# google-deepmind/pycolab

Hardware: NVIDIA H100
Metric: env_steps_per_sec (higher is better)
Workload: dtype u8

## Files before the change

pycolab_b200/csrc/pcl_kernels.cuh:

```cuda
#pragma once

#include <cuda_runtime.h>
#include <stdint.h>
#include <string.h>

#include "../../include/pcl.h"

namespace pcl {

struct CropParams {
  int B, H, W, pitch, S;
  pcl_crop_spec crop;
  const int32_t* sprites;
  int32_t* plot;
  int32_t* state;
  const uint8_t* board;
  uint8_t* out;
  const uint8_t* curtains[PCL_MAX_TRACK];
  uint32_t cols_recip;
};

struct StepParams {
  int B, H, W, pitch;
  int PH, PW, PWW;
  int BW;
  int S, D;
  int auto_reset;
  int mode;
  int actions_per_env;
  int margin[PCL_MAX_DRAPES][2];
  uint8_t sprite_char[PCL_MAX_SPRITES];
  uint8_t drape_char[PCL_MAX_DRAPES];
  uint32_t impassable[PCL_MAX_SPRITES][4];
  int confined[PCL_MAX_SPRITES];
  int egocentric[PCL_MAX_SPRITES];
  int drape_kind[PCL_MAX_DRAPES];
  int program_arg[8];
  int n_scroll_groups;
  int sprite_group[PCL_MAX_SPRITES];
  int drape_group[PCL_MAX_DRAPES];
  int n_groups;
  int group_len[PCL_MAX_SPRITES + PCL_MAX_DRAPES];
  uint8_t group_chars[PCL_MAX_SPRITES + PCL_MAX_DRAPES];
  pcl_state st;
  pcl_outputs out;
  const int32_t* actions;
  const uint8_t* env_mask;
  int has_cropper;
  CropParams cropper;
  const int32_t* code;
  uint8_t* backdrop_live;
  const uint32_t* derived[2];
  int64_t derived_bstride[2];
  int32_t* render_key;
  uint32_t board_epoch;
};

template <typename... Params, typename... Args>
cudaError_t launch_pdl(void (*kern)(Params...), int grid, int block, size_t smem, cudaStream_t s,
                       Args... args) {
  cudaLaunchConfig_t cfg = {};
  cfg.gridDim = dim3(grid); cfg.blockDim = dim3(block); cfg.dynamicSmemBytes = smem; cfg.stream = s;
  cudaLaunchAttribute attr[1];
  attr[0].id = cudaLaunchAttributeProgrammaticStreamSerialization;
  attr[0].val.programmaticStreamSerializationAllowed = 1;
  cfg.attrs = attr; cfg.numAttrs = 1;
  return cudaLaunchKernelEx(&cfg, kern, args...);
}

inline cudaError_t launch_step(void (*kern)(StepParams), const StepParams& p, int warps,
                               size_t smem, cudaStream_t s, bool pdl = false) {
  if (smem > 48 * 1024) {
    cudaError_t e = cudaFuncSetAttribute(kern, cudaFuncAttributeMaxDynamicSharedMemorySize, (int)smem);
    if (e != cudaSuccess) return e;
  }
  const int grid = (p.B + warps - 1) / warps;
  if (pdl) return launch_pdl(kern, grid, warps * 32, smem, s, p);
  kern<<<grid, warps * 32, smem, s>>>(p);
  return cudaGetLastError();
}

enum class CurtainAt { kNone, kBits, kPatternWindow, kStaleWindow };

struct Program {
  int (*check_spec)(const pcl_spec&);
  int (*check_state)(const pcl_spec&, const pcl_state&);
  CurtainAt (*curtain)(const pcl_spec&, int drape);
  cudaError_t (*launch)(const StepParams&, cudaStream_t);
  int (*actions_per_env)(const pcl_spec&);
  bool float_reward;
  bool crop_epilogue;
  bool scroll_groups;
  int (*check_code)(const pcl_spec&, const int32_t* words, int n_words);
  bool float_reward_arg0;
  int (*derive)(const pcl_spec&, const pcl_state&, int batch, StepParams* base, void** owned);
};
extern const Program kScrollyMaze, kWarehouse, kMarauders, kFixture, kBetterScrolly, kClassics,
    kAperture, kOrdeal, kHello, kApprehend, kShockwave, kTMaze, kCompiled, kBoxWorld,
    kCuedCatch, kSequenceRecall;

inline bool chars_are(const uint8_t* got, int n, const char* want) {
  if ((int)strlen(want) != n) return false;
  for (int i = 0; i < n; ++i) if (got[i] != (uint8_t)want[i]) return false;
  return true;
}

inline bool set_is(const uint32_t (&got)[4], const char* want) {
  uint32_t m[4] = {0, 0, 0, 0};
  for (const char* c = want; *c; ++c) m[(*c >> 5) & 3] |= 1u << (*c & 31);
  return m[0] == got[0] && m[1] == got[1] && m[2] == got[2] && m[3] == got[3];
}

inline int groups_are(const pcl_spec& s, const char* flat, const int* lens, int n) {
  if (s.n_groups != n) return 0;
  int k = 0;
  for (int g = 0; g < n; ++g) {
    if (s.group_len[g] != lens[g]) return 0;
    for (int i = 0; i < lens[g]; ++i, ++k)
      if (s.group_chars[k] != (uint8_t)flat[k]) return 0;
  }
  return 1;
}

inline bool bit_rows_fit(const pcl_spec& s) { return s.bits_words >= (s.cols + 31) / 32 + 1; }

inline bool margins_fit(const pcl_spec& s, int d) {
  const int mr = s.margins[d][0], mc = s.margins[d][1];
  return !(mr >= 0 && (mc - 1 >= s.cols - mc || mr - 1 >= s.rows - mr));
}

inline CurtainAt curtain_bits(const pcl_spec&, int) { return CurtainAt::kBits; }

struct RenderParams {
  int B, H, W, pitch, S, D;
  const uint8_t* backdrop; int64_t backdrop_bstride;
  const uint8_t* curtains;
  const int32_t* sprites;
  const uint8_t* z_order;
  uint8_t sprite_char[PCL_MAX_SPRITES];
  uint8_t drape_char[PCL_MAX_DRAPES];
  uint8_t* board;
};
cudaError_t launch_render(const RenderParams& p, cudaStream_t s);

#define PCL_MAX_LAYER_CHARS 32
struct LayersParams {
  int B, H, W, pitch, S, D, n_chars;
  uint8_t chars[PCL_MAX_LAYER_CHARS];
  int8_t sprite_of[PCL_MAX_LAYER_CHARS];
  int8_t drape_of[PCL_MAX_LAYER_CHARS];
  const uint32_t* bits[PCL_MAX_DRAPES]; int64_t bits_bstride[PCL_MAX_DRAPES];
  int row_words[PCL_MAX_DRAPES];
  int scrolly[PCL_MAX_DRAPES];
  int per_level[PCL_MAX_DRAPES];
  int stale_slot[PCL_MAX_DRAPES];
  const uint8_t* backdrop; int64_t backdrop_bstride;
  const int32_t* level;
  const int32_t* sprites;
  const int32_t* drapes;
  uint8_t* out;
  int backdrop_per_env;
};
cudaError_t launch_layers(const LayersParams& p, cudaStream_t s);

struct ObserveParams {
  int B, H, W, pitch, depth, dtype;
  int words;
  int64_t stride_b, stride_d, stride_r, stride_c;
  const void* table;
  const uint8_t* valid;
  const uint8_t* board;
  void* out;
  int32_t* unknown;
};
cudaError_t launch_observe(const ObserveParams& p, cudaStream_t s);

cudaError_t launch_crop(const CropParams& p, cudaStream_t s);

struct HandoffParams {
  int n_peers, rank, record_bytes;
  int64_t rows;
  int64_t first_row;
  uint8_t* peer_base[PCL_MAX_PEERS];
  uint32_t* peer_flags[PCL_MAX_PEERS];
  uint8_t* multicast;
  uint32_t* local;
  int n_bufs, lag;
  int signal_kernel;
  pcl_outputs out;
};
cudaError_t launch_crop_handoff(const CropParams& p, const HandoffParams& x, cudaStream_t s);

struct PackParams {
  int B, view_bytes, record_bytes;
  const uint8_t* view;
  pcl_outputs out;
  uint8_t* packed;
  int n_peers;
  int64_t first_row;
  uint8_t* peers[PCL_MAX_PEERS];
};
cudaError_t launch_pack_handoff(const PackParams& p, cudaStream_t s);

}
```

pycolab_b200/csrc/scrolly_maze.cu:

```cuda
#include <algorithm>
#include <new>

#include "pcl_device.cuh"
#include "pcl_kernels.cuh"
#include "pcl_crop.cuh"

namespace pcl {

namespace {

constexpr int kS = 4;
constexpr int kWarpsPerBlock = 4;
constexpr int kRecWords = 64;

__device__ __forceinline__ int action_to_motion(int a) {
  constexpr unsigned kTable = (PCL_M_N) | (PCL_M_S << 4) | (PCL_M_W << 8) | (PCL_M_E << 12) |
                              (PCL_M_STAY << 16);
  return (unsigned)a < 5u ? (int)((kTable >> (4 * a)) & 15u) : PCL_M_NONE;
}

__device__ __forceinline__ void cp_async8(void* smem, const void* gmem) {
  asm volatile("cp.async.ca.shared.global [%0], [%1], 8;\n" ::
               "r"((uint32_t)__cvta_generic_to_shared(smem)), "l"(gmem));
}
__device__ __forceinline__ void cp_async16_l1(void* smem, const void* gmem) {
  asm volatile("cp.async.ca.shared.global [%0], [%1], 16;\n" ::
               "r"((uint32_t)__cvta_generic_to_shared(smem)), "l"(gmem));
}


__device__ __forceinline__ int coin_group_shift(int PH) {
  return 32 - __clz((PH - 1) >> 5);
}

__device__ __forceinline__ uint32_t prmt(uint32_t a, uint32_t b, uint32_t sel) {
  uint32_t d;
  asm("prmt.b32 %0, %1, %2, %3;" : "=r"(d) : "r"(a), "r"(b), "r"(sel));
  return d;
}

__host__ __device__ constexpr int window_words(int W) {
  return W < 2 ? 4 : 2 * ((63 + W + 63) / 64);
}

__host__ __device__ constexpr bool narrow_board(int pitch) { return pitch <= 64; }

constexpr int kKeyStride = 16;
enum { kKeyRecWords = 8, kKeyEpoch = 8, kKeySprites = 9, kKeyWords = kKeySprites + kS };
constexpr uint64_t kKeyRec =
    (uint64_t)(48 + PCL_P_FRAME) | (uint64_t)(32 + PCL_D_CORNER_R) << 8 |
    (uint64_t)(32 + PCL_D_CORNER_C) << 16 | (uint64_t)(40 + PCL_D_CORNER_R) << 24 |
    (uint64_t)(40 + PCL_D_CORNER_C) << 32 | (uint64_t)(40 + PCL_D_AUX0) << 40 |
    (uint64_t)(40 + PCL_D_AUX1) << 48 | (uint64_t)(40 + PCL_D_AUX2) << 56;
static_assert(kKeyWords <= kKeyStride, "the render key outgrew its slot");

enum {
  kNbWall = 0,
  kNbCoin = 32,
  kNbBackdrop = 44,
  kNbStart = 56,
  kNbStale = kNbStart + 4 * kS,
  kNbWords = (kNbStale + 2 + 3) & ~3
};

__host__ __device__ constexpr size_t staging_bytes(int H, int W, int pitch) {
  return (size_t)H * pitch + 2 * ((((size_t)H * window_words(W) * 4) + 15) & ~(size_t)15) +
         (narrow_board(pitch) ? 0 : (((size_t)H * (pitch >> 2) + 15) & ~(size_t)15));
}

__host__ __device__ constexpr size_t warp_smem_bytes(int H, int W, int pitch) {
  return kRecWords * 4 + (staging_bytes(H, W, pitch) > (size_t)kNbWords * 4
                             ? staging_bytes(H, W, pitch) : (size_t)kNbWords * 4);
}

__device__ __forceinline__ void pdl_launch_dependents() {
  asm volatile("griddepcontrol.launch_dependents;" ::: "memory");
}
__device__ __forceinline__ void pdl_wait_prior_grids() {
  asm volatile("griddepcontrol.wait;" ::: "memory");
}

struct SelTable { uint16_t v[256]; };
constexpr SelTable make_sel_table() {
  SelTable t = {};
  for (int idx = 0; idx < 256; ++idx) {
    unsigned sel = 0;
    for (int k = 0; k < 4; ++k) {
      const unsigned nib = ((idx >> (4 + k)) & 1) ? 5u : ((idx >> k) & 1) ? 4u : (unsigned)k;
      sel |= nib << (4 * k);
    }
    t.v[idx] = (uint16_t)sel;
  }
  return t;
}
__device__ __align__(16) const SelTable g_sel = make_sel_table();

#ifdef PCL_STEP_STAMPS
constexpr int kStampEnvs = 8192;
enum {
  kStEntry, kStPrior, kStRecords, kStPatch, kStGroup2, kStWait, kStPatched, kStPaint, kStEnd,
  kStTimeIn, kStTimeOut, kStPath, kStampWords
};
enum { kPathDelta, kPathDeltaPickup, kPathFellBack, kPathFull, kPathRestart };
__device__ uint32_t g_stamps[kStampEnvs][kStampWords];
__device__ __forceinline__ uint32_t global_ns() {
  uint32_t t;
  asm volatile("mov.u32 %0, %%globaltimer_lo;" : "=r"(t));
  return t;
}
__device__ __forceinline__ void stamp(int k, uint32_t v) {
  uint32_t tid, cta;
  asm volatile("mov.u32 %0, %%tid.x;" : "=r"(tid));
  asm volatile("mov.u32 %0, %%ctaid.x;" : "=r"(cta));
  const uint32_t e = cta * kWarpsPerBlock + (tid >> 5);
  if ((tid & 31) == 0 && e < (uint32_t)kStampEnvs) g_stamps[e][k] = v;
}
#define PCL_STAMP(k) stamp(k, (uint32_t)clock())
#define PCL_STAMP_TIME(k) stamp(k, global_ns())
#define PCL_STAMP_PATH(v) stamp(kStPath, (uint32_t)(v))
#else
#define PCL_STAMP(k) do {} while (0)
#define PCL_STAMP_TIME(k) do {} while (0)
#define PCL_STAMP_PATH(v) do {} while (0)
#endif

constexpr size_t kMaxBlockSmem = 227 * 1024 - 2048;

static_assert(8 * (kWarpsPerBlock * (warp_smem_bytes(64, 64, 64) + sizeof(SelTable)) + 1024) <=
                  228 * 1024,
              "a 64x64 scrolly_maze block no longer fits 8 times per SM");
static_assert(warp_smem_bytes(1, 1, 16) == kRecWords * 4 + kNbWords * 4,
              "delta rendering's scratch must fit a warp's region on the smallest board");
static_assert(kMaxBlockSmem + kWarpsPerBlock * sizeof(SelTable) == 227 * 1024,
              "kMaxBlockSmem must leave room for the static selector tables");

__device__ __forceinline__ unsigned blocked3x3(int vrow, int vcol, int r0, int c0, unsigned field,
                                               int H, int W, bool p_vis, int p_row, int p_col) {
  const int br = vrow - r0 + 1, bc = vcol - c0 + 1;
  if ((unsigned)br > 2u || (unsigned)bc > 2u) return 0u;
  unsigned colmask = 0;
#pragma unroll
  for (int i = 0; i < 3; ++i) colmask |= ((unsigned)(vcol - 1 + i) < (unsigned)W ? 1u : 0u) << i;
  unsigned blk = 0;
#pragma unroll
  for (int j = 0; j < 3; ++j) {
    unsigned bits = (field >> ((br + j) * 5 + bc)) & colmask;
    if ((unsigned)(vrow - 1 + j) >= (unsigned)H) bits = 0;
    blk |= bits << (3 * j);
  }
  const int dr = p_row - vrow + 1, dc = p_col - vcol + 1;
  if (p_vis && (unsigned)dr <= 2u && (unsigned)dc <= 2u) blk &= ~(1u << (dr * 3 + dc));
  return blk;
}

__device__ __forceinline__ int legal_motions(unsigned b) {
  const unsigned nw = b & 1u, n = (b >> 1) & 1u, ne = (b >> 2) & 1u, w = (b >> 3) & 1u,
                 e = (b >> 5) & 1u, sw = (b >> 6) & 1u, s = (b >> 7) & 1u, se = (b >> 8) & 1u;
  const unsigned blocked = n | ((ne | (n & e)) << 1) | (e << 2) | ((se | (s & e)) << 3) |
                           (s << 4) | ((sw | (s & w)) << 5) | (w << 6) | ((nw | (n & w)) << 7);
  return (int)((~blocked & 0xffu) | (1u << PCL_M_STAY));
}

__device__ __forceinline__ void scrolly_move_p(Drape& d, const ScrollyCfg& cfg, int motion,
                                               Plot& plot, int p_row, int p_col, int p_permit,
                                               int p_permit_frame) {
  if (d.last_frame < plot.frame) {
    d.last_frame = plot.frame;
    d.pre_r = d.corner_r; d.pre_c = d.corner_c;
  }
  const int dr = motion_dr(motion), dc = motion_dc(motion);
  if (plot.order_frame == plot.frame) {
    if (dr != plot.order_r && dc != plot.order_c) plot.error |= PCL_ENV_ERR_ORDER_MISMATCH;
    d.corner_r += plot.order_r; d.corner_c += plot.order_c;
    return;
  }
  if (motion == PCL_M_STAY) return;
  const bool ego = plot.ego_mask & 1;
  const bool possible = !ego || (p_permit_frame == plot.frame && ((p_permit >> motion) & 1));
  int orr, occ;
  if (!cfg.have_margins) {
    if (!possible) return;
    const int nr = d.corner_r + dr, nc = d.corner_c + dc;
    orr = (0 <= nr && nr <= cfg.limit_r) ? dr : 0;
    occ = (0 <= nc && nc <= cfg.limit_c) ? dc : 0;
  } else {
    if (!ego) return;
    const int nr = p_row + dr, nc = p_col + dc;
    const bool want_v = (p_row > nr && nr <= cfg.m_north) || (p_row < nr && nr >= cfg.m_south);
    const bool want_h = (p_col > nc && nc <= cfg.m_west) || (p_col < nc && nc >= cfg.m_east);
    if (!(want_v || want_h)) return;
    orr = want_v ? dr : 0; occ = want_h ? dc : 0;
    const int cr = d.corner_r + orr, cc = d.corner_c + occ;
    if (!((0 <= cr && cr <= cfg.limit_r) && (0 <= cc && cc <= cfg.limit_c)) || !possible) return;
  }
  d.corner_r += orr; d.corner_c += occ;
  plot.order_r = orr; plot.order_c = occ; plot.order_frame = plot.frame;
}

__device__ __forceinline__ int64_t level_of(const StepParams& p, int env) {
  return p.st.d_level ? p.st.d_level[env] : env;
}
__device__ __forceinline__ const uint32_t* level_walls(const StepParams& p, int64_t lvl) {
  return p.st.d_pattern[0] + lvl * p.st.pattern_bstride[0];
}
__device__ __forceinline__ uint32_t* env_coins(const StepParams& p, int env) {
  return p.st.d_pattern[1] + (int64_t)env * p.st.pattern_bstride[1];
}
__device__ __forceinline__ const uint32_t* level_coins(const StepParams& p, int64_t lvl) {
  return p.st.d_pattern_init[1] + lvl * p.st.pattern_init_bstride[1];
}

__device__ __forceinline__ int32_t key_word(const int32_t* rec, int i, uint32_t epoch, int pitch) {
  const int32_t r = rec[i < kKeyRecWords ? (int)((kKeyRec >> (8 * i)) & 0xffu) : 0];
  const int32_t* q = rec + min(max(i - kKeySprites, 0), kS - 1) * PCL_SPRITE_WORDS;
  const int32_t cell = q[PCL_S_FLAGS] & 1 ? q[PCL_S_ROW] * pitch + q[PCL_S_COL] : -1;
  return i < kKeyRecWords ? r : i == kKeyEpoch ? (int32_t)epoch : cell;
}

__global__ void __launch_bounds__(kWarpsPerBlock * 32, 8)
scrolly_maze_step(const StepParams p) {
  extern __shared__ __align__(16) uint8_t smem_raw[];
  PCL_STAMP(kStEntry);
  PCL_STAMP_TIME(kStTimeIn);
  __shared__ __align__(16) uint16_t s_sel_all[kWarpsPerBlock][256];
  const int lane = threadIdx.x & 31;
  const int warp = threadIdx.x >> 5;
  uint16_t* s_sel = s_sel_all[warp];
  pdl_launch_dependents();
  const int env = blockIdx.x * kWarpsPerBlock + warp;
  const bool live = env < p.B;
  const int H = p.H, W = p.W, PWW = p.PWW;
  const int pitch = p.pitch;
  const int nw = window_words(W);

  uint8_t* my = smem_raw + warp * warp_smem_bytes(H, W, pitch);
  int32_t* rec = reinterpret_cast<int32_t*>(my);
  uint8_t* s_bd = my + kRecWords * 4;
  uint32_t* s_wall = reinterpret_cast<uint32_t*>(s_bd + (size_t)H * pitch);
  uint32_t* s_coin = s_wall + ((H * nw + 3) & ~3);
  pdl_wait_prior_grids();
  PCL_STAMP(kStPrior);
  if (p.has_cropper && p.cropper.state && live && lane == 0)
    asm volatile("prefetch.global.L2 [%0];" :: "l"(p.cropper.state + (int64_t)env * 4));
  if (!live) return;
  const int64_t lvl = level_of(p, env);

  int action = env_action(p, env);
  const int32_t key = lane < kKeyWords ? p.render_key[(int64_t)env * kKeyStride + lane] : 0;
  rec[lane] = p.st.d_sprites[(int64_t)env * kS * PCL_SPRITE_WORDS + lane];
  rec[32 + lane] = lane < 16 ? p.st.d_drapes[(int64_t)env * 2 * PCL_DRAPE_WORDS + lane]
                             : p.st.d_plot[(int64_t)env * PCL_PLOT_WORDS + lane - 16];
  __syncwarp();
  PCL_STAMP(kStRecords);
  const int was_over = rec[48 + PCL_P_GAME_OVER];
  bool restart;
  bool frozen = false;
  if (p.mode == MODE_RESET) {
    restart = (p.env_mask == nullptr) || (p.env_mask[env] != 0);
    frozen = !restart;
  } else {
    restart = was_over && p.auto_reset;
    frozen = was_over && !p.auto_reset;
  }
  if (frozen) return;
  const bool key_ok = __all_sync(PCL_FULL, lane >= kKeyWords ||
                                               key == key_word(rec, lane, p.board_epoch, pitch));
  if (restart) {
    const PlotCarry carry = plot_carry(rec + 48, true);
    const unsigned dirty = p.mode == MODE_RESET ? ~0u
                                                : (unsigned)rec[32 + PCL_DRAPE_WORDS + PCL_D_AUX2];
    __syncwarp();
    const int32_t* si = p.st.d_sprites_init + lvl * p.st.sprites_init_bstride;
    const int32_t* di = p.st.d_drapes_init + lvl * p.st.drapes_init_bstride;
    const int32_t* pi = p.st.d_plot_init + lvl * p.st.plot_init_bstride;
    rec[lane] = __ldg(si + lane);
    rec[32 + lane] = lane < 16 ? __ldg(di + lane) : __ldg(pi + lane - 16);
    const uint32_t* src = level_coins(p, lvl);
    const int n = p.PH * PWW, gw = PWW << coin_group_shift(p.PH);
    for (unsigned m = dirty; m != 0u; m &= m - 1u) {
      const int lo = (__ffs(m) - 1) * gw, hi = min(lo + gw, n);
      for (int i = lo + lane; i < hi; i += 32) env_coins(p, env)[i] = __ldg(src + i);
    }
    __syncwarp();
    if (lane == 0) store_carry(rec + 48, carry);
    __syncwarp();
    action = PCL_ACTION_NONE;
  }

  const int me = lane & 3;
  Sprite mine;
  {
    const int32_t* r = rec + me * PCL_SPRITE_WORDS;
    mine.row = r[PCL_S_ROW]; mine.col = r[PCL_S_COL];
    mine.vrow = r[PCL_S_VROW]; mine.vcol = r[PCL_S_VCOL];
    mine.flags = r[PCL_S_FLAGS]; mine.aux0 = r[PCL_S_AUX0]; mine.aux1 = r[PCL_S_AUX1];
    mine.aux2 = 0;
  }
  const int p_row = rec[PCL_S_ROW], p_col = rec[PCL_S_COL];
  const int p_vrow = rec[PCL_S_VROW], p_vcol = rec[PCL_S_VCOL];
  const bool p_vis = rec[PCL_S_FLAGS] & 1;
  const int p_permit = rec[PCL_S_AUX0], p_permit_frame = rec[PCL_S_AUX1];
  const int32_t* rec_coins = rec + 32 + PCL_DRAPE_WORDS;
  Drape walls;
  {
    const int32_t* r = rec + 32;
    walls.corner_r = r[PCL_D_CORNER_R]; walls.corner_c = r[PCL_D_CORNER_C];
    walls.pre_r = r[PCL_D_PRE_R]; walls.pre_c = r[PCL_D_PRE_C];
    walls.last_frame = r[PCL_D_LAST_FRAME];
  }
  Plot plot;
  {
    const int32_t* r = rec + 48;
    plot.frame = r[PCL_P_FRAME]; plot.error = r[PCL_P_ERROR];
    plot.order_r = r[PCL_P_ORDER_R]; plot.order_c = r[PCL_P_ORDER_C];
    plot.order_frame = r[PCL_P_ORDER_FRAME]; plot.ego_mask = r[PCL_P_EGO_MASK];
  }

  const ScrollyCfg wcfg = scrolly_cfg(H, W, p.PH, p.PW, p.margin[0][0], p.margin[0][1]);
  const ScrollyCfg ccfg = scrolly_cfg(H, W, p.PH, p.PW, p.margin[1][0], p.margin[1][1]);
  Directives dir = fresh_directives();
  const int motion = action_to_motion(action);

  plot.frame += 1;

  if (motion != PCL_M_NONE)
    scrolly_move_p(walls, wcfg, motion, plot, p_row, p_col, p_permit, p_permit_frame);
  const bool ordered = plot.order_frame == plot.frame;
  const int wr = walls.corner_r, wc = walls.corner_c;
  const int cr_pred = rec_coins[PCL_D_CORNER_R] + (ordered && motion != PCL_M_NONE ? plot.order_r : 0);
  const int cc_pred = rec_coins[PCL_D_CORNER_C] + (ordered && motion != PCL_M_NONE ? plot.order_c : 0);

  const int we = (wc >> 5) & ~1, ce = (cc_pred >> 5) & ~1;
  const bool narrow = narrow_board(pitch);
  const bool c_touch = rec_coins[PCL_D_LAST_FRAME] < plot.frame;
  const int c_pre_r = rec_coins[c_touch ? PCL_D_CORNER_R : PCL_D_PRE_R];
  const int c_pre_c = rec_coins[c_touch ? PCL_D_CORNER_C : PCL_D_PRE_C];
  unsigned rowbits = 0;
  {
    const uint32_t* row = nullptr;
    int c_first = 0, limit = 0;
    if (lane < 20) {
      const int w = lane / 5, k = lane - w * 5;
      const int pr = wr + rec[w * PCL_SPRITE_WORDS + PCL_S_VROW] + k - 2;
      c_first = wc + rec[w * PCL_SPRITE_WORDS + PCL_S_VCOL] - 2;
      if ((unsigned)pr < (unsigned)p.PH) { row = level_walls(p, lvl) + (int64_t)pr * PWW; limit = PWW; }
    } else if (lane < 24) {
      const int r = lane < 23 ? p_vrow + (lane - 20) - 1 : 0;
      c_first = lane < 23 ? c_pre_c + p_vcol - 1 : c_pre_c;
      if ((unsigned)r < (unsigned)H) {
        const int pr = c_pre_r + r;
        row = ((unsigned)rec_coins[PCL_D_AUX2] >> (pr >> coin_group_shift(p.PH))) & 1u
                  ? env_coins(p, env) : level_coins(p, lvl);
        row += (int64_t)pr * PWW; limit = PWW;
      }
    }
    if (row != nullptr) {
      const int wi = c_first >> 5;
      const uint32_t lo = (unsigned)wi < (unsigned)limit ? row[wi] : 0u;
      const uint32_t hi = (unsigned)(wi + 1) < (unsigned)limit ? row[wi + 1] : 0u;
      rowbits = __funnelshift_r(lo, hi, c_first & 31) & 31u;
    }
  }
  bool delta = key_ok && !restart && wr == rec[32 + PCL_D_CORNER_R] &&
               wc == rec[32 + PCL_D_CORNER_C] && cr_pred == rec_coins[PCL_D_CORNER_R] &&
               cc_pred == rec_coins[PCL_D_CORNER_C] && rec_coins[PCL_D_AUX2] != -1;
  unsigned nb = 0;
  if (delta && lane < 24) {
    const int s = (lane < 12 ? lane : lane - 12) / 3;
    const int vr = rec[s * PCL_SPRITE_WORDS + PCL_S_VROW], vc = rec[s * PCL_SPRITE_WORDS + PCL_S_VCOL];
    const int r = vr + (lane < 12 ? lane : lane - 12) - 3 * s - 1;
    if ((unsigned)r < (unsigned)H) {
      if (lane < 12) {
        const int pr = cr_pred + r, c_first = cc_pred + vc - 1, wi = c_first >> 5;
        const uint32_t* row = ((unsigned)rec_coins[PCL_D_AUX2] >> (pr >> coin_group_shift(p.PH))) & 1u
                                  ? env_coins(p, env) : level_coins(p, lvl);
        row += (int64_t)pr * PWW;
        const uint32_t lo = (unsigned)wi < (unsigned)PWW ? row[wi] : 0u;
        const uint32_t hi = (unsigned)(wi + 1) < (unsigned)PWW ? row[wi + 1] : 0u;
        nb = __funnelshift_r(lo, hi, c_first & 31) & 7u;
      } else {
        const uint8_t* bd = p.st.d_backdrop + lvl * p.st.backdrop_bstride + (int64_t)r * pitch;
#pragma unroll
        for (int j = 0; j < 3; ++j)
          if ((unsigned)(vc - 1 + j) < (unsigned)W) nb |= (unsigned)__ldg(bd + vc - 1 + j) << (8 * j);
      }
    }
  }
  unsigned field = 0;
#pragma unroll
  for (int k = 0; k < 5; ++k) field |= __shfl_sync(PCL_FULL, rowbits, me * 5 + k) << (5 * k);
  unsigned coin9 = 0;
  {
    unsigned colmask = 0;
#pragma unroll
    for (int i = 0; i < 3; ++i)
      colmask |= ((unsigned)(p_vcol - 1 + i) < (unsigned)W ? 1u : 0u) << i;
#pragma unroll
    for (int k = 0; k < 3; ++k) coin9 |= (__shfl_sync(PCL_FULL, rowbits, 20 + k) & colmask) << (3 * k);
    coin9 |= (__shfl_sync(PCL_FULL, rowbits, 23) & 1u) << 9;
  }
  PCL_STAMP(kStPatch);
  uint32_t* s_nb = reinterpret_cast<uint32_t*>(s_bd);
  auto stage = [&](int64_t lvl) {
    cp_async16_l1(reinterpret_cast<uint8_t*>(s_sel) + lane * 16,
                  reinterpret_cast<const uint8_t*>(g_sel.v) + lane * 16);
    {
      const uint8_t* src = p.st.d_backdrop + lvl * p.st.backdrop_bstride + lane * 16;
      uint8_t* dst = s_bd + lane * 16;
      const int n16 = (H * pitch) >> 4;
#pragma unroll 4
      for (int i = lane; i < n16; i += 32, src += 512, dst += 512) cp_async16(dst, src);
    }
    {
      const int gs = coin_group_shift(p.PH);
      const uint32_t* wsrc =
          p.derived[0] + lvl * p.derived_bstride[0] + ((int64_t)(we >> 1) * p.PH + wr) * nw;
      const uint32_t* csrc =
          p.derived[1] + lvl * p.derived_bstride[1] + ((int64_t)(ce >> 1) * p.PH + cr_pred) * nw;
      const int hw = nw >> 1, nhalf = H * hw;
      if (narrow) {
#pragma unroll 1
        for (int r = lane; r < H; r += 32) {
          cp_async16(s_wall + r * 4, wsrc + r * 4);
          if (!(((unsigned)rec_coins[PCL_D_AUX2] >> ((cr_pred + r) >> gs)) & 1u))
            cp_async16(s_coin + r * 4, csrc + r * 4);
        }
      } else {
#pragma unroll 1
        for (int i = lane; i < nhalf; i += 32) {
          const int pr = cr_pred + i / hw;
          cp_async8(s_wall + i * 2, wsrc + i * 2);
          if (!(((unsigned)rec_coins[PCL_D_AUX2] >> (pr >> gs)) & 1u))
            cp_async8(s_coin + i * 2, csrc + i * 2);
        }
      }
      if (rec_coins[PCL_D_AUX2] != 0) {
#pragma unroll 1
        for (int i = lane; i < nhalf; i += 32) {
          const int r = narrow ? i >> 1 : i / hw, k = (i - r * hw) * 2, pr = cr_pred + r;
          if (((unsigned)rec_coins[PCL_D_AUX2] >> (pr >> gs)) & 1u)
            cp_async8(s_coin + i * 2, env_coins(p, env) + (int64_t)pr * PWW + ce + k);
        }
      }
    }
  };
  if (delta) {
    if (lane < 20) s_nb[kNbWall + lane] = rowbits;
    if (lane < 24) s_nb[kNbCoin + lane] = nb;
    if (lane < 4) {
      uint32_t* q = s_nb + kNbStart + 4 * lane;
      q[0] = mine.vrow; q[1] = mine.vcol;
      q[2] = visible(mine) ? mine.row : -1; q[3] = mine.col;
    }
    if (lane < 2) s_nb[kNbStale + lane] = rec_coins[PCL_D_AUX0 + lane];
  } else {
    stage(lvl);
    PCL_STAMP_PATH(restart ? kPathRestart : kPathFull);
  }

  const int r0 = mine.vrow, c0 = mine.vcol;
  const bool is_p = me == 0;
  const bool even = (plot.frame % 2) == 0;
  if (even) scrolly_touch_prescroll(walls, plot);
  int my_err = 0;
  bool hit = false;
  int mot;
  if (is_p) {
    mot = motion;
  } else if (!even) {
    mot = PCL_M_STAY;
  } else {
    const int step = mine.aux0 ? 1 : -1;
    int pr = r0 + walls.pre_r, pc = c0 + walls.pre_c + step;
    bool next_to_wall = false;
    if ((unsigned)pr < (unsigned)p.PH && (unsigned)pc < (unsigned)p.PW) {
      const int dr = pr - wr - r0 + 2, dc = pc - wc - c0 + 2;
      next_to_wall = (field >> (dr * 5 + dc)) & 1u;
    } else {
      if (pr < 0) pr += p.PH;
      if (pc < 0) pc += p.PW;
      if ((unsigned)pr < (unsigned)p.PH && (unsigned)pc < (unsigned)p.PW)
        next_to_wall = bit_at(level_walls(p, level_of(p, env)) + (int64_t)pr * PWW, pc);
      else
        my_err |= PCL_ENV_ERR_INDEX;
    }
    if (next_to_wall) mine.aux0 = !mine.aux0;
    mot = mine.aux0 ? PCL_M_E : PCL_M_W;
  }
  if (mot != PCL_M_NONE) {
    const int dr = motion_dr(mot), dc = motion_dc(mot);
    if (ordered) {
      walker_teleport(mine, H, W, mine.vrow - plot.order_r, mine.vcol - plot.order_c);
      if (is_p && plot.order_r != dr && plot.order_c != dc) my_err |= PCL_ENV_ERR_ORDER_MISMATCH;
    }
    bool legal = true;
    unsigned blk = 0;
    if (mot != PCL_M_STAY || is_p) {
      blk = blocked3x3(mine.vrow, mine.vcol, r0, c0, field, H, W, p_vis, p_row, p_col);
      legal = motion_legal(blk, mot);
    }
    if (legal && mot != PCL_M_STAY) {
      walker_teleport(mine, H, W, mine.vrow + dr, mine.vcol + dc);
      if (is_p) blk = blocked3x3(mine.vrow, mine.vcol, r0, c0, field, H, W, p_vis, p_row, p_col);
    }
    if (is_p) {
      const int valid_at = plot.frame + 1;
      if (mine.aux1 != valid_at) { mine.aux1 = valid_at; mine.aux0 = 0; }
      mine.aux0 |= legal_motions(blk);
    } else if (even) {
      hit = mine.vrow == p_vrow && mine.vcol == p_vcol;
    }
  }
  __syncwarp();
  if (lane < 4) {
    int32_t* r = rec + me * PCL_SPRITE_WORDS;
    r[PCL_S_ROW] = mine.row; r[PCL_S_COL] = mine.col;
    r[PCL_S_VROW] = mine.vrow; r[PCL_S_VCOL] = mine.vcol;
    r[PCL_S_FLAGS] = mine.flags; r[PCL_S_AUX0] = mine.aux0;
    if (is_p) r[PCL_S_AUX1] = mine.aux1;
  }
  if (motion != PCL_M_NONE) plot.ego_mask |= 1;
  plot.error |= __reduce_or_sync(PCL_FULL, (unsigned)(lane < 4 ? my_err : 0));
  if (__any_sync(PCL_FULL, lane < 4 && hit)) terminate(dir);
  Sprite pl;
  pl.row = __shfl_sync(PCL_FULL, mine.row, 0); pl.col = __shfl_sync(PCL_FULL, mine.col, 0);
  pl.vrow = __shfl_sync(PCL_FULL, mine.vrow, 0); pl.vcol = __shfl_sync(PCL_FULL, mine.vcol, 0);
  pl.flags = __shfl_sync(PCL_FULL, mine.flags, 0);
  pl.aux0 = __shfl_sync(PCL_FULL, mine.aux0, 0); pl.aux1 = __shfl_sync(PCL_FULL, mine.aux1, 0);

  Drape coins;
  coins.corner_r = rec_coins[PCL_D_CORNER_R]; coins.corner_c = rec_coins[PCL_D_CORNER_C];
  coins.pre_r = rec_coins[PCL_D_PRE_R]; coins.pre_c = rec_coins[PCL_D_PRE_C];
  coins.last_frame = rec_coins[PCL_D_LAST_FRAME];
  coins.aux0 = rec_coins[PCL_D_AUX0]; coins.aux1 = rec_coins[PCL_D_AUX1];
  scrolly_touch_prescroll(coins, plot);
  plot.aux0 = rec[48 + PCL_P_AUX0];
  int picked_r = -1, picked_c = -1;
  {
    const int dr = pl.row - p_vrow, dc = pl.col - p_vcol;
    bool coin;
    const int pr = coins.pre_r + pl.row, pc = coins.pre_c + pl.col;
    if (pl.row == 0 && pl.col == 0 && !on_board(pl.vrow, pl.vcol, H, W))
      coin = (coin9 >> 9) & 1u;
    else if ((unsigned)(dr + 1) <= 2u && (unsigned)(dc + 1) <= 2u)
      coin = (coin9 >> ((dr + 1) * 3 + dc + 1)) & 1u;
    else
      coin = bit_at(env_coins(p, env) + (int64_t)pr * PWW, pc);
    if (coin) {
      add_reward(dir, 100);
      if (lane == 0) atomicAnd(env_coins(p, env) + (int64_t)pr * PWW + (pc >> 5), ~(1u << (pc & 31)));
      picked_r = pr; picked_c = pc;
      plot.aux0 -= 1;
      if (plot.aux0 == 0) terminate(dir);
      coins.aux0 = pl.row; coins.aux1 = pl.col;
    }
  }
  if (motion != PCL_M_NONE) {
    scrolly_move_p(coins, ccfg, motion, plot, pl.row, pl.col, pl.aux0, pl.aux1);
    coins.aux0 = -1; coins.aux1 = -1;
  } else if (action == 5) {
    terminate(dir);
  }
  PCL_STAMP(kStGroup2);

  cp_async_wait_all();
  PCL_STAMP(kStWait);
  __syncwarp();
  if (lane == 0) {
    int32_t* r = rec + 32;
    r[PCL_D_CORNER_R] = walls.corner_r; r[PCL_D_CORNER_C] = walls.corner_c;
    r[PCL_D_PRE_R] = walls.pre_r; r[PCL_D_PRE_C] = walls.pre_c;
    r[PCL_D_LAST_FRAME] = walls.last_frame;
    r += PCL_DRAPE_WORDS;
    r[PCL_D_CORNER_R] = coins.corner_r; r[PCL_D_CORNER_C] = coins.corner_c;
    r[PCL_D_PRE_R] = coins.pre_r; r[PCL_D_PRE_C] = coins.pre_c;
    r[PCL_D_LAST_FRAME] = coins.last_frame;
    r[PCL_D_AUX0] = coins.aux0; r[PCL_D_AUX1] = coins.aux1;
    r = rec + 48;
    r[PCL_P_FRAME] = plot.frame; r[PCL_P_GAME_OVER] = dir.game_over;
    r[PCL_P_ERROR] = plot.error;
    r[PCL_P_ORDER_R] = plot.order_r; r[PCL_P_ORDER_C] = plot.order_c;
    r[PCL_P_ORDER_FRAME] = plot.order_frame; r[PCL_P_EGO_MASK] = plot.ego_mask;
    r[PCL_P_AUX0] = plot.aux0;
    store_outputs(p.out, env, dir);
    if (picked_r >= 0) rec[32 + PCL_DRAPE_WORDS + PCL_D_AUX2] |= 1 << (picked_r >> coin_group_shift(p.PH));
  }
  const int cr = coins.corner_r, cc = coins.corner_c;

  if (delta) {
    __syncwarp();
    bool fall = cr != cr_pred || cc != cc_pred;
    int cell = -1;
    uint32_t val = 0;
    if (!fall) {
      int r = -1, c = -1;
      if (lane < 4) {
        r = (int)s_nb[kNbStart + 4 * lane + 2]; c = (int)s_nb[kNbStart + 4 * lane + 3];
      } else if (lane < 8) {
        const int32_t* s = rec + (lane - 4) * PCL_SPRITE_WORDS;
        if (s[PCL_S_FLAGS] & 1) { r = s[PCL_S_ROW]; c = s[PCL_S_COL]; }
      } else if (lane == 8) {
        r = (int)s_nb[kNbStale]; c = (int)s_nb[kNbStale + 1];
      } else if (lane == 9) {
        r = rec_coins[PCL_D_AUX0]; c = rec_coins[PCL_D_AUX1];
      } else if (lane == 10 && picked_r >= 0) {
        r = picked_r - cr; c = picked_c - cc;
      }
      bool outside = false;
      if (r >= 0) {
        int s = -1, dr = 0, dc = 0;
#pragma unroll
        for (int t = kS - 1; t >= 0; --t) {
          const int a = r - (int)s_nb[kNbStart + 4 * t] + 1, b = c - (int)s_nb[kNbStart + 4 * t + 1] + 1;
          if ((unsigned)a <= 2u && (unsigned)b <= 2u) { s = t; dr = a; dc = b; }
        }
        outside = s < 0 || !on_board(r, c, H, W);
        if (!outside) {
          const bool wall = (s_nb[kNbWall + 5 * s + dr + 1] >> (dc + 1)) & 1u;
          bool coin = (s_nb[kNbCoin + 3 * s + dr] >> dc) & 1u;
          if (picked_r - cr == r && picked_c - cc == c) coin = false;
          if (rec_coins[PCL_D_AUX0] == r && rec_coins[PCL_D_AUX1] == c) coin = true;
          val = (s_nb[kNbBackdrop + 3 * s + dr] >> (8 * dc)) & 0xffu;
#pragma unroll
          for (int t = 1; t <= kS; ++t) {
            const int32_t* q = rec + (t & 3) * PCL_SPRITE_WORDS;
            if (t == kS && coin) val = '@';
            if (t == kS && wall) val = '#';
            if ((q[PCL_S_FLAGS] & 1) && q[PCL_S_ROW] == r && q[PCL_S_COL] == c) val = p.sprite_char[t & 3];
          }
          cell = r * pitch + c;
        }
      }
      fall = __any_sync(PCL_FULL, outside);
    }
    if (fall) {
      __syncwarp();
      delta = false;
      stage(level_of(p, env));
      cp_async_wait_all();
      PCL_STAMP_PATH(kPathFellBack);
    } else if (cell >= 0) {
      p.out.d_board[(int64_t)env * H * pitch + cell] = (uint8_t)val;
    }
  }

  if (!delta && lane == 0 && picked_r >= 0) {
    const int r2 = picked_r - cr_pred, b = picked_c - (ce << 5);
    if ((unsigned)r2 < (unsigned)H && (unsigned)b < (unsigned)(nw * 32))
      s_coin[r2 * nw + (b >> 5)] &= ~(1u << (b & 31));
  }
  int ce_final = ce;
  if (cr != cr_pred || cc != cc_pred) {
    __syncwarp();
    ce_final = (cc >> 5) & ~1;
    for (int i = lane; i < H * nw; i += 32)
      s_coin[i] = env_coins(p, env)[(int64_t)(cr + i / nw) * PWW + ce_final + i % nw];
  }
  __syncwarp();
  p.st.d_sprites[(int64_t)env * kS * PCL_SPRITE_WORDS + lane] = rec[lane];
  if (lane < 16) p.st.d_drapes[(int64_t)env * 2 * PCL_DRAPE_WORDS + lane] = rec[32 + lane];
  else p.st.d_plot[(int64_t)env * PCL_PLOT_WORDS + lane - 16] = rec[32 + lane];
  if (lane < kKeyWords)
    p.render_key[(int64_t)env * kKeyStride + lane] = key_word(rec, lane, p.board_epoch, pitch);
  if (delta) {
    PCL_STAMP_PATH(picked_r >= 0 ? kPathDeltaPickup : kPathDelta);
    PCL_STAMP(kStPatched);
    PCL_STAMP(kStPaint);
    if (p.has_cropper) {
      __syncwarp();
      crop_epilogue(p.cropper, p.out.d_board, env, lane, rec, rec + 48);
    }
    PCL_STAMP(kStEnd);
    PCL_STAMP_TIME(kStTimeOut);
    return;
  }

  const int spr = pitch >> 4;
  uint32_t* s_seg = narrow ? s_wall : s_coin + ((H * nw + 3) & ~3);
  const int wsh = wc - (we << 5), csh = cc - (ce_final << 5);
  if (narrow) {
    const uint32_t m_lo = W >= 32 ? 0xffffffffu : (1u << W) - 1u;
    const uint32_t m_hi = W >= 64 ? 0xffffffffu : W > 32 ? (1u << (W - 32)) - 1u : 0u;
    for (int r0 = 0; r0 < H; r0 += 32) {
      const int r = min(r0 + lane, H - 1);
      const uint4 wv = *reinterpret_cast<const uint4*>(s_wall + r * 4);
      const uint4 cv = *reinterpret_cast<const uint4*>(s_coin + r * 4);
      const uint32_t wa = (wsh & 32) ? wv.y : wv.x, wb = (wsh & 32) ? wv.z : wv.y,
                     wd = (wsh & 32) ? wv.w : wv.z;
      const uint32_t ca = (csh & 32) ? cv.y : cv.x, cb = (csh & 32) ? cv.z : cv.y,
                     cd = (csh & 32) ? cv.w : cv.z;
      const uint32_t w_lo = __funnelshift_r(wa, wb, wsh & 31) & m_lo;
      const uint32_t w_hi = __funnelshift_r(wb, wd, wsh & 31) & m_hi;
      const uint32_t c_lo = __funnelshift_r(ca, cb, csh & 31) & m_lo;
      const uint32_t c_hi = __funnelshift_r(cb, cd, csh & 31) & m_hi;
      __syncwarp();
      if (r0 + lane < H) {
        uint32_t* out = s_seg + r * spr;
        out[0] = __byte_perm(c_lo, w_lo, 0x5410);
        if (spr > 1) out[1] = __byte_perm(c_lo, w_lo, 0x7632);
        if (spr > 2) out[2] = __byte_perm(c_hi, w_hi, 0x5410);
        if (spr > 3) out[3] = __byte_perm(c_hi, w_hi, 0x7632);
      }
    }
  } else {
    for (int i = lane; i < H * spr; i += 32) {
      const int r = i / spr, j = i - r * spr;
      const int ncols = min(16, W - 16 * j);
      if (ncols <= 0) { s_seg[i] = 0; continue; }
      const uint32_t keep = (1u << ncols) - 1u;
      const int wo = wsh + 16 * j, co = csh + 16 * j;
      const uint32_t* wrow = s_wall + r * nw;
      const uint32_t* crow = s_coin + r * nw;
      const uint32_t w16 = __funnelshift_r(wrow[wo >> 5], (wo >> 5) + 1 < nw ? wrow[(wo >> 5) + 1] : 0u,
                                           wo & 31) & keep;
      const uint32_t c16 = __funnelshift_r(crow[co >> 5], (co >> 5) + 1 < nw ? crow[(co >> 5) + 1] : 0u,
                                           co & 31) & keep;
      s_seg[i] = (w16 << 16) | c16;
    }
  }
  __syncwarp();
  if (lane == 0 && coins.aux0 >= 0)
    s_seg[coins.aux0 * spr + (coins.aux1 >> 4)] |= 1u << (coins.aux1 & 15);
#pragma unroll
  for (int i = 1; i < kS; ++i) {
    if (lane == i && visible(mine)) s_bd[mine.row * pitch + mine.col] = p.sprite_char[i];
    __syncwarp();
  }
  if (lane == 0 && visible(pl)) {
    s_bd[pl.row * pitch + pl.col] = p.sprite_char[0];
    s_seg[pl.row * spr + (pl.col >> 4)] &= ~(0x00010001u << (pl.col & 15));
  }
  __syncwarp();
  PCL_STAMP(kStPatched);
  const int total = H * spr;
  const unsigned drape_chars = ('#' << 8) | '@';
  const uint4* src = reinterpret_cast<const uint4*>(s_bd);
  uint4* dst = reinterpret_cast<uint4*>(p.out.d_board + (int64_t)env * H * pitch);
  for (int seg = lane; seg < total; seg += 32) {
    uint4 px = src[seg];
    const uint32_t bits = s_seg[seg];
    px.x = prmt(px.x, drape_chars, s_sel[((bits >> 12) & 0xf0u) | (bits & 0xfu)]);
    px.y = prmt(px.y, drape_chars, s_sel[((bits >> 16) & 0xf0u) | ((bits >> 4) & 0xfu)]);
    px.z = prmt(px.z, drape_chars, s_sel[((bits >> 20) & 0xf0u) | ((bits >> 8) & 0xfu)]);
    px.w = prmt(px.w, drape_chars, s_sel[((bits >> 24) & 0xf0u) | ((bits >> 12) & 0xfu)]);
    dst[seg] = px;
  }
  PCL_STAMP(kStPaint);
  if (p.has_cropper) {
    __syncwarp();
    crop_epilogue(p.cropper, p.out.d_board, env, lane, rec, rec + 48);
  }
  PCL_STAMP(kStEnd);
  PCL_STAMP_TIME(kStTimeOut);
}

size_t block_smem(int H, int W, int pitch) {
  return warp_smem_bytes(H, W, pitch) * kWarpsPerBlock;
}

int check_spec(const pcl_spec& s) {
  if (!chars_are(s.sprite_char, s.n_sprites, "Pabc")) return PCL_ERR_UNSUPPORTED;
  if (!chars_are(s.drape_char, s.n_drapes, "#@")) return PCL_ERR_UNSUPPORTED;
  if (!chars_are(s.z_order, 6, "abc@#P")) return PCL_ERR_UNSUPPORTED;
  const int lens[3] = {1, 4, 1};
  if (!groups_are(s, "#abcP@", lens, 3)) return PCL_ERR_UNSUPPORTED;
  for (int i = 0; i < 4; ++i) {
    if (!set_is(s.impassable[i], "#")) return PCL_ERR_UNSUPPORTED;
    if (s.sprite_confined[i]) return PCL_ERR_UNSUPPORTED;
    if (s.sprite_egocentric[i] != (i == 0)) return PCL_ERR_UNSUPPORTED;
  }
  if (s.pattern_rows < s.rows || s.pattern_cols < s.cols) return PCL_ERR_INVALID;
  {
    const int nw = window_words(s.cols);
    if ((s.pattern_words & 1) || s.pattern_words < (((s.pattern_cols - s.cols) >> 5) & ~1) + nw ||
        s.pattern_words < (s.pattern_cols + 31) / 32 + 1) return PCL_ERR_INVALID;
    if (block_smem(s.rows, s.cols, s.pitch) > kMaxBlockSmem) return PCL_ERR_UNSUPPORTED;
  }
  for (int d = 0; d < 2; ++d)
    if (!margins_fit(s, d)) return PCL_ERR_INVALID;
  return PCL_OK;
}

int check_state(const pcl_spec&, const pcl_state& st) {
  for (int d = 0; d < 2; ++d) if (!st.d_pattern[d]) return PCL_ERR_INVALID;
  if (!st.d_pattern_init[1] || st.pattern_bstride[1] == 0) return PCL_ERR_INVALID;
  return PCL_OK;
}

CurtainAt curtain(const pcl_spec&, int d) {
  return d == 1 ? CurtainAt::kStaleWindow : CurtainAt::kPatternWindow;
}

cudaError_t launch(const StepParams& p, cudaStream_t s) {
  if (p.PWW & 1) return cudaErrorInvalidValue;
  const size_t smem = block_smem(p.H, p.W, p.pitch);
  if (smem > kMaxBlockSmem) return cudaErrorInvalidValue;
  return launch_step(scrolly_maze_step, p, kWarpsPerBlock, smem, s, true);
}


__global__ void build_blocked(const uint32_t* src, int64_t src_bstride, uint32_t* dst, int PH,
                              int PWW, int nw, int nblk, int64_t total) {
  for (int64_t i = blockIdx.x * (int64_t)blockDim.x + threadIdx.x; i < total;
       i += (int64_t)gridDim.x * blockDim.x) {
    int64_t t = i / nw;
    const int w = (int)(i - t * nw);
    const int row = (int)(t % PH);
    t /= PH;
    const int k = (int)(t % nblk);
    dst[i] = src[(t / nblk) * src_bstride + (int64_t)row * PWW + 2 * k + w];
  }
}

int derive(const pcl_spec& s, const pcl_state& st, int batch, StepParams* p, void** owned) {
  int64_t levels = batch;
  if (st.d_level) {
    int32_t* lv = new (std::nothrow) int32_t[batch];
    if (!lv) return PCL_ERR_NOMEM;
    const cudaError_t e = cudaMemcpy(lv, st.d_level, sizeof(int32_t) * batch, cudaMemcpyDeviceToHost);
    levels = 1;
    for (int i = 0; e == cudaSuccess && i < batch; ++i) levels = std::max<int64_t>(levels, lv[i] + 1);
    delete[] lv;
    if (e != cudaSuccess) return PCL_ERR_CUDA;
  }
  const int W = s.cols, PH = s.pattern_rows;
  const int nw = window_words(W), nblk = ((((s.pattern_cols - W) >> 5) & ~1) >> 1) + 1;
  const int64_t blk_words = (int64_t)nblk * PH * nw;
  const int64_t n_wall = st.pattern_bstride[0] == 0 ? 1 : levels;
  const int64_t n_coin = st.pattern_init_bstride[1] == 0 ? 1 : levels;
  const int64_t off_coin = (n_wall * blk_words * 4 + 255) & ~(int64_t)255;
  const int64_t off_key = (off_coin + n_coin * blk_words * 4 + 255) & ~(int64_t)255;
  uint8_t* buf = nullptr;
  if (cudaMalloc(&buf, off_key + (int64_t)batch * kKeyStride * 4) != cudaSuccess) return PCL_ERR_NOMEM;
  *owned = buf;
  uint32_t* wall = reinterpret_cast<uint32_t*>(buf);
  uint32_t* coin = reinterpret_cast<uint32_t*>(buf + off_coin);
  p->render_key = reinterpret_cast<int32_t*>(buf + off_key);
  if (cudaMemset(p->render_key, 0xff, (size_t)batch * kKeyStride * 4) != cudaSuccess) return PCL_ERR_CUDA;
  build_blocked<<<1024, 256>>>(st.d_pattern[0], st.pattern_bstride[0], wall, PH, s.pattern_words,
                               nw, nblk, n_wall * blk_words);
  build_blocked<<<1024, 256>>>(st.d_pattern_init[1], st.pattern_init_bstride[1], coin, PH,
                               s.pattern_words, nw, nblk, n_coin * blk_words);
  p->derived[0] = wall; p->derived_bstride[0] = n_wall > 1 ? blk_words : 0;
  p->derived[1] = coin; p->derived_bstride[1] = n_coin > 1 ? blk_words : 0;
  return cudaDeviceSynchronize() == cudaSuccess && cudaGetLastError() == cudaSuccess ? PCL_OK
                                                                                     : PCL_ERR_CUDA;
}

}

const Program kScrollyMaze = {check_spec, check_state, curtain, launch, nullptr,
                              false, true,
                              false, nullptr,
                              false, derive};

}

#ifdef PCL_STEP_STAMPS
extern "C" int pcl_step_stamps(uint32_t* host, int n) {
  if (n < 0 || n > pcl::kStampEnvs) return -1;
  return cudaMemcpyFromSymbol(host, pcl::g_stamps, sizeof(pcl::g_stamps[0]) * n) == cudaSuccess
             ? 0 : -3;
}
#endif
```

Measured before the change: 467.2 million.

## Precompute 5x5 wall neighbourhood words and merge patch gathers into one load pass

Adds a derived table holding, for every pattern cell, a packed 25-bit 5x5 wall neighbourhood, built once at setup. The step kernel then fetches each sprite's wall patch with one word load instead of five row loads plus funnel shifts per lane. It also folds the coin and backdrop neighbourhood gathers into the same single lane-parallel load with evict_last L2 hints, which removes one of the gather phases and the five-shuffle field assembly. In exchange it uses extra device memory sized to the padded pattern per level, and the loads are always issued rather than only on the delta path.

```diff
diff --git a/pycolab_b200/csrc/pcl_kernels.cuh b/pycolab_b200/csrc/pcl_kernels.cuh
--- a/pycolab_b200/csrc/pcl_kernels.cuh
+++ b/pycolab_b200/csrc/pcl_kernels.cuh
@@ -50,8 +50,8 @@
   CropParams cropper;
   const int32_t* code;
   uint8_t* backdrop_live;
-  const uint32_t* derived[2];
-  int64_t derived_bstride[2];
+  const uint32_t* derived[3];
+  int64_t derived_bstride[3];
   int32_t* render_key;
   uint32_t board_epoch;
 };
diff --git a/pycolab_b200/csrc/scrolly_maze.cu b/pycolab_b200/csrc/scrolly_maze.cu
--- a/pycolab_b200/csrc/scrolly_maze.cu
+++ b/pycolab_b200/csrc/scrolly_maze.cu
@@ -26,6 +26,17 @@
 __device__ __forceinline__ void cp_async16_l1(void* smem, const void* gmem) {
   asm volatile("cp.async.ca.shared.global [%0], [%1], 16;\n" ::
                "r"((uint32_t)__cvta_generic_to_shared(smem)), "l"(gmem));
+}
+
+__device__ __forceinline__ uint64_t l2_evict_last() {
+  uint64_t policy;
+  asm("createpolicy.fractional.L2::evict_last.b64 %0, 1.0;" : "=l"(policy));
+  return policy;
+}
+__device__ __forceinline__ uint32_t ld_keep(const uint32_t* p, uint64_t policy) {
+  uint32_t v;
+  asm volatile("ld.global.L2::cache_hint.u32 %0, [%1], %2;" : "=r"(v) : "l"(p), "l"(policy) : "memory");
+  return v;
 }
 
 
@@ -62,6 +73,7 @@
   kNbStale = kNbStart + 4 * kS,
   kNbWords = (kNbStale + 2 + 3) & ~3
 };
+static_assert(kNbBackdrop == kNbCoin + 12, "the patch trip stores coin and backdrop rows as one run");
 
 __host__ __device__ constexpr size_t staging_bytes(int H, int W, int pitch) {
   return (size_t)H * pitch + 2 * ((((size_t)H * window_words(W) * 4) + 15) & ~(size_t)15) +
@@ -335,60 +347,48 @@
   const bool c_touch = rec_coins[PCL_D_LAST_FRAME] < plot.frame;
   const int c_pre_r = rec_coins[c_touch ? PCL_D_CORNER_R : PCL_D_PRE_R];
   const int c_pre_c = rec_coins[c_touch ? PCL_D_CORNER_C : PCL_D_PRE_C];
-  unsigned rowbits = 0;
-  {
-    const uint32_t* row = nullptr;
-    int c_first = 0, limit = 0;
-    if (lane < 20) {
-      const int w = lane / 5, k = lane - w * 5;
-      const int pr = wr + rec[w * PCL_SPRITE_WORDS + PCL_S_VROW] + k - 2;
-      c_first = wc + rec[w * PCL_SPRITE_WORDS + PCL_S_VCOL] - 2;
-      if ((unsigned)pr < (unsigned)p.PH) { row = level_walls(p, lvl) + (int64_t)pr * PWW; limit = PWW; }
-    } else if (lane < 24) {
-      const int r = lane < 23 ? p_vrow + (lane - 20) - 1 : 0;
-      c_first = lane < 23 ? c_pre_c + p_vcol - 1 : c_pre_c;
-      if ((unsigned)r < (unsigned)H) {
-        const int pr = c_pre_r + r;
-        row = ((unsigned)rec_coins[PCL_D_AUX2] >> (pr >> coin_group_shift(p.PH))) & 1u
-                  ? env_coins(p, env) : level_coins(p, lvl);
-        row += (int64_t)pr * PWW; limit = PWW;
-      }
-    }
-    if (row != nullptr) {
-      const int wi = c_first >> 5;
-      const uint32_t lo = (unsigned)wi < (unsigned)limit ? row[wi] : 0u;
-      const uint32_t hi = (unsigned)(wi + 1) < (unsigned)limit ? row[wi + 1] : 0u;
-      rowbits = __funnelshift_r(lo, hi, c_first & 31) & 31u;
-    }
-  }
   bool delta = key_ok && !restart && wr == rec[32 + PCL_D_CORNER_R] &&
                wc == rec[32 + PCL_D_CORNER_C] && cr_pred == rec_coins[PCL_D_CORNER_R] &&
                cc_pred == rec_coins[PCL_D_CORNER_C] && rec_coins[PCL_D_AUX2] != -1;
-  unsigned nb = 0;
-  if (delta && lane < 24) {
-    const int s = (lane < 12 ? lane : lane - 12) / 3;
+  uint32_t got;
+  {
+    const bool wall_lane = lane < 4, coin_lane = lane < 20, pc_lane = lane < 8;
+    const int j = coin_lane ? lane - 8 : lane - 20;
+    const int s = wall_lane ? lane : pc_lane ? 0 : j / 3;
     const int vr = rec[s * PCL_SPRITE_WORDS + PCL_S_VROW], vc = rec[s * PCL_SPRITE_WORDS + PCL_S_VCOL];
-    const int r = vr + (lane < 12 ? lane : lane - 12) - 3 * s - 1;
-    if ((unsigned)r < (unsigned)H) {
-      if (lane < 12) {
-        const int pr = cr_pred + r, c_first = cc_pred + vc - 1, wi = c_first >> 5;
-        const uint32_t* row = ((unsigned)rec_coins[PCL_D_AUX2] >> (pr >> coin_group_shift(p.PH))) & 1u
-                                  ? env_coins(p, env) : level_coins(p, lvl);
-        row += (int64_t)pr * PWW;
-        const uint32_t lo = (unsigned)wi < (unsigned)PWW ? row[wi] : 0u;
-        const uint32_t hi = (unsigned)(wi + 1) < (unsigned)PWW ? row[wi + 1] : 0u;
-        nb = __funnelshift_r(lo, hi, c_first & 31) & 7u;
-      } else {
-        const uint8_t* bd = p.st.d_backdrop + lvl * p.st.backdrop_bstride + (int64_t)r * pitch;
+    const int r = pc_lane ? (lane < 7 ? p_vrow + lane - 5 : 0) : vr + j - 3 * (j / 3) - 1;
+    const int c = pc_lane ? (lane < 7 ? c_pre_c + p_vcol - 1 : c_pre_c)
+                          : coin_lane ? cc_pred + vc - 1 : vc - 1;
+    const bool row_ok = (unsigned)r < (unsigned)H && (pc_lane || delta);
+    const int pr = (pc_lane ? c_pre_r : cr_pred) + r;
+    const uint32_t* coin_row =
+        (((unsigned)rec_coins[PCL_D_AUX2] >> (pr >> coin_group_shift(p.PH))) & 1u
+             ? env_coins(p, env) : level_coins(p, lvl)) + (int64_t)pr * PWW;
+    const int wr_c = wr + vr + 2, wc_c = wc + vc + 2;
+    const int tw = p.PW + 4;
+    const uint32_t* base =
+        wall_lane ? p.derived[2] + lvl * p.derived_bstride[2] + (int64_t)wr_c * tw + wc_c
+        : coin_lane ? coin_row
+                    : reinterpret_cast<const uint32_t*>(p.st.d_backdrop + lvl * p.st.backdrop_bstride +
+                                                        (int64_t)r * pitch);
+    const int words = coin_lane ? PWW : pitch >> 2;
+    const int wi = wall_lane ? 0 : coin_lane ? c >> 5 : c >> 2;
+    const bool ok0 = wall_lane ? (unsigned)wr_c < (unsigned)(p.PH + 4) && (unsigned)wc_c < (unsigned)tw
+                               : row_ok && (unsigned)wi < (unsigned)words;
+    const bool ok1 = !wall_lane && row_ok && (unsigned)(wi + 1) < (unsigned)words;
+    const int sh = wall_lane ? 0 : coin_lane ? c & 31 : (c & 3) * 8;
+    uint32_t mask = wall_lane ? ~0u : lane == 7 ? 1u : 7u;
+    if (!coin_lane) {
+      mask = 0;
 #pragma unroll
-        for (int j = 0; j < 3; ++j)
-          if ((unsigned)(vc - 1 + j) < (unsigned)W) nb |= (unsigned)__ldg(bd + vc - 1 + j) << (8 * j);
-      }
-    }
-  }
-  unsigned field = 0;
-#pragma unroll
-  for (int k = 0; k < 5; ++k) field |= __shfl_sync(PCL_FULL, rowbits, me * 5 + k) << (5 * k);
+      for (int i = 0; i < 3; ++i) mask |= ((unsigned)(c + i) < (unsigned)W ? 0xffu : 0u) << (8 * i);
+    }
+    const uint64_t keep = l2_evict_last();
+    const uint32_t lo = ok0 ? ld_keep(base + wi, keep) : 0u;
+    const uint32_t hi = ok1 ? ld_keep(base + wi + 1, keep) : 0u;
+    got = __funnelshift_r(lo, hi, sh) & mask;
+  }
+  const unsigned field = __shfl_sync(PCL_FULL, got, me);
   unsigned coin9 = 0;
   {
     unsigned colmask = 0;
@@ -396,8 +396,8 @@
     for (int i = 0; i < 3; ++i)
       colmask |= ((unsigned)(p_vcol - 1 + i) < (unsigned)W ? 1u : 0u) << i;
 #pragma unroll
-    for (int k = 0; k < 3; ++k) coin9 |= (__shfl_sync(PCL_FULL, rowbits, 20 + k) & colmask) << (3 * k);
-    coin9 |= (__shfl_sync(PCL_FULL, rowbits, 23) & 1u) << 9;
+    for (int k = 0; k < 3; ++k) coin9 |= (__shfl_sync(PCL_FULL, got, 4 + k) & colmask) << (3 * k);
+    coin9 |= __shfl_sync(PCL_FULL, got, 7) << 9;
   }
   PCL_STAMP(kStPatch);
   uint32_t* s_nb = reinterpret_cast<uint32_t*>(s_bd);
@@ -445,8 +445,8 @@
     }
   };
   if (delta) {
-    if (lane < 20) s_nb[kNbWall + lane] = rowbits;
-    if (lane < 24) s_nb[kNbCoin + lane] = nb;
+    if (lane < 4) s_nb[kNbWall + lane] = got;
+    if (lane >= 8) s_nb[kNbCoin + lane - 8] = got;
     if (lane < 4) {
       uint32_t* q = s_nb + kNbStart + 4 * lane;
       q[0] = mine.vrow; q[1] = mine.vcol;
@@ -616,7 +616,7 @@
         }
         outside = s < 0 || !on_board(r, c, H, W);
         if (!outside) {
-          const bool wall = (s_nb[kNbWall + 5 * s + dr + 1] >> (dc + 1)) & 1u;
+          const bool wall = (s_nb[kNbWall + s] >> ((dr + 1) * 5 + dc + 1)) & 1u;
           bool coin = (s_nb[kNbCoin + 3 * s + dr] >> dc) & 1u;
           if (picked_r - cr == r && picked_c - cc == c) coin = false;
           if (rec_coins[PCL_D_AUX0] == r && rec_coins[PCL_D_AUX1] == c) coin = true;
@@ -812,6 +812,29 @@
   }
 }
 
+__global__ void build_neighbourhoods(const uint32_t* src, int64_t src_bstride, uint32_t* dst, int PH,
+                                     int PW, int PWW, int64_t total) {
+  const int tw = PW + 4;
+  const int64_t per_copy = (int64_t)(PH + 4) * tw;
+  for (int64_t i = blockIdx.x * (int64_t)blockDim.x + threadIdx.x; i < total;
+       i += (int64_t)gridDim.x * blockDim.x) {
+    const int64_t t = i / per_copy;
+    const int cell = (int)(i - t * per_copy);
+    const int pr = cell / tw - 2, c_first = cell % tw - 4;
+    const int wi = c_first >> 5;
+    uint32_t word = 0;
+    for (int k = 0; k < 5; ++k) {
+      const int r = pr + k - 2;
+      if ((unsigned)r >= (unsigned)PH) continue;
+      const uint32_t* row = src + t * src_bstride + (int64_t)r * PWW;
+      const uint32_t lo = (unsigned)wi < (unsigned)PWW ? row[wi] : 0u;
+      const uint32_t hi = (unsigned)(wi + 1) < (unsigned)PWW ? row[wi + 1] : 0u;
+      word |= (__funnelshift_r(lo, hi, c_first & 31) & 31u) << (5 * k);
+    }
+    dst[i] = word;
+  }
+}
+
 int derive(const pcl_spec& s, const pcl_state& st, int batch, StepParams* p, void** owned) {
   int64_t levels = batch;
   if (st.d_level) {
@@ -828,21 +851,27 @@
   const int64_t blk_words = (int64_t)nblk * PH * nw;
   const int64_t n_wall = st.pattern_bstride[0] == 0 ? 1 : levels;
   const int64_t n_coin = st.pattern_init_bstride[1] == 0 ? 1 : levels;
+  const int64_t nbh_words = (int64_t)(PH + 4) * (s.pattern_cols + 4);
   const int64_t off_coin = (n_wall * blk_words * 4 + 255) & ~(int64_t)255;
-  const int64_t off_key = (off_coin + n_coin * blk_words * 4 + 255) & ~(int64_t)255;
+  const int64_t off_nbh = (off_coin + n_coin * blk_words * 4 + 255) & ~(int64_t)255;
+  const int64_t off_key = (off_nbh + n_wall * nbh_words * 4 + 255) & ~(int64_t)255;
   uint8_t* buf = nullptr;
   if (cudaMalloc(&buf, off_key + (int64_t)batch * kKeyStride * 4) != cudaSuccess) return PCL_ERR_NOMEM;
   *owned = buf;
   uint32_t* wall = reinterpret_cast<uint32_t*>(buf);
   uint32_t* coin = reinterpret_cast<uint32_t*>(buf + off_coin);
+  uint32_t* nbh = reinterpret_cast<uint32_t*>(buf + off_nbh);
   p->render_key = reinterpret_cast<int32_t*>(buf + off_key);
   if (cudaMemset(p->render_key, 0xff, (size_t)batch * kKeyStride * 4) != cudaSuccess) return PCL_ERR_CUDA;
   build_blocked<<<1024, 256>>>(st.d_pattern[0], st.pattern_bstride[0], wall, PH, s.pattern_words,
                                nw, nblk, n_wall * blk_words);
   build_blocked<<<1024, 256>>>(st.d_pattern_init[1], st.pattern_init_bstride[1], coin, PH,
                                s.pattern_words, nw, nblk, n_coin * blk_words);
+  build_neighbourhoods<<<1024, 256>>>(st.d_pattern[0], st.pattern_bstride[0], nbh, PH,
+                                      s.pattern_cols, s.pattern_words, n_wall * nbh_words);
   p->derived[0] = wall; p->derived_bstride[0] = n_wall > 1 ? blk_words : 0;
   p->derived[1] = coin; p->derived_bstride[1] = n_coin > 1 ? blk_words : 0;
+  p->derived[2] = nbh; p->derived_bstride[2] = n_wall > 1 ? nbh_words : 0;
   return cudaDeviceSynchronize() == cudaSuccess && cudaGetLastError() == cudaSuccess ? PCL_OK
                                                                                      : PCL_ERR_CUDA;
 }
@@ -854,6 +883,13 @@
                               false, nullptr,
                               false, derive};
 
+}
+
+extern "C" int pcl_scrolly_wall_neighbourhoods(const uint32_t* d_pattern, int64_t bstride, int rows,
+                                               int cols, int words, int64_t copies, uint32_t* d_dst) {
+  pcl::build_neighbourhoods<<<1024, 256>>>(d_pattern, bstride, d_dst, rows, cols, words,
+                                           copies * (rows + 4) * (cols + 4));
+  return cudaDeviceSynchronize() == cudaSuccess && cudaGetLastError() == cudaSuccess ? 0 : -3;
 }
 
 #ifdef PCL_STEP_STAMPS
```

Result: faster. 492.2 million (median of 6 runs) (+5.3%).
